# HengyiWang/MorpheuS

Hardware: AMD Instinct MI355X
Metric: rays/sec (fwd+bwd, 128 samples/ray) (higher is better)
Workload: dtype f32 (exact 3 x bf16 operand split on the bf16 MFMA pipe, fp32 accumulate)

## Files before the change

include/morpheus_hip.h:

```cpp
#ifndef MORPHEUS_HIP_H
#define MORPHEUS_HIP_H

#include <stdint.h>

#ifdef __cplusplus
extern "C" {
#endif

#define MH_OK 0
#define MH_ERR_ARG 1
#define MH_ERR_LAUNCH 2
#define MH_ERR_OVERFLOW 3

#define MH_ABI_VERSION 9
#define MH_MAX_LEVELS 32
#define MH_TILE 32

int mh_abi_version(void);
const char *mh_status_string(int status);

int mh_grid_encode_fwd(const float *x, const float *emb, const int32_t *offsets_host,
                       const int32_t *res_host, float *out, int64_t M, int32_t L, int32_t n_levels,
                       float bound, int32_t group, void *stream);
int mh_grid_encode_bwd(const float *grad, const float *x, const float *emb,
// ... 116 lines not shown
int64_t mh_field_wpackT_floats(void);
int mh_field_fwd(const float *xc, const float *feat_s, const float *feat_c, const float *topo,
                 const float *wpack, const float *bias, const float *beta, int32_t n_bands, int32_t with_color,
                 float *sdf, float *sigma, float *albedo, float *acts, int64_t M, void *stream);
int64_t mh_mlp_wgrad_workspace_floats(int32_t n_layers, const int32_t *in_feats_host,
                                      const int32_t *out_feats_host, int64_t n_tiles);
int mh_mlp_wgrad(const float *acts, const float *dpre, int64_t acts_tile_floats, int64_t dpre_tile_floats,
                 int32_t n_layers, const int32_t *act_off_host, const int32_t *dpre_off_host,
                 const int32_t *in_feats_host, const int32_t *out_feats_host, const int32_t *in_live_host,
                 const int32_t *out_live_host, float *workspace, float *dw_raw, float *db_raw, int64_t n_tiles, void *stream);
int mh_mlp_wgrad_b3(const float *acts, const float *dpre, int64_t acts_tile_floats, int64_t dpre_tile_floats,
                    int32_t n_layers, const int32_t *act_off_host, const int32_t *dpre_off_host,
                    const int32_t *in_feats_host, const int32_t *out_feats_host, const int32_t *in_live_host,
                    const int32_t *out_live_host, float *workspace, float *dw_raw, float *db_raw, int64_t n_tiles, void *stream);

int mh_weight_norm_fwd(int32_t n_layers, const float *const *v_host, const float *const *g_host, float *const *w_host,
                       const int32_t *rows_host, const int32_t *cols_host, void *stream);
int mh_weight_norm_bwd(int32_t n_layers, const float *const *v_host, const float *const *g_host,
                       const float *const *dw_host, float *const *dv_host, float *const *dg_host,
                       const int32_t *rows_host, const int32_t *cols_host, void *stream);

int64_t mh_field_bwd_fused_workspace_floats(int64_t M);
int64_t mh_field_dgeo_floats(int64_t M);
int mh_field_bwd_fused(const float *xc, const float *sdf, const float *albedo, const float *g_sdf, const float *g_sigma,
                       const float *g_albedo, const float *wpackT, const float *beta, int32_t n_bands, int32_t with_color,
                       const float *acts, float *dgeo_scratch, float *workspace, float *raw, int32_t accumulate, float *g_xc,
                       float *g_feat_s, float *g_feat_c, float *g_topo, uint32_t *gmax_bits, int64_t M, void *stream);
int64_t mh_field_w3T_bytes(void);
int mh_field_bwd_fused_b3(const float *xc, const float *sdf, const float *albedo, const float *g_sdf, const float *g_sigma,
                          const float *g_albedo, const void *w3T, const float *beta, int32_t n_bands, int32_t with_color,
                          const float *acts, float *dgeo_scratch, float *workspace, float *raw, int32_t accumulate, float *g_xc,
                          float *g_feat_s, float *g_feat_c, float *g_topo, uint32_t *gmax_bits, int64_t M, void *stream);
int64_t mh_field_bwd_pair_min_points(int64_t set);
int mh_adam_step(float *params, const float *grads, float *exp_avg, float *exp_avg_sq, int64_t n, int32_t n_segs,
                 const int64_t *seg_end_host, const float *seg_lr_host, const int64_t *seg_step_host, float beta1,
                 float beta2, float eps, void *stream);
int mh_adam_step_dev(float *params, const float *grads, float *exp_avg, float *exp_avg_sq, int64_t n, int32_t n_segs,
                     const int64_t *seg_end_host, const float *seg_lr_host, const float *seg_flag_dev, int64_t *seg_step_dev,
                     float *seg_scratch_dev, float beta1, float beta2, float eps, void *stream);

int64_t mh_masked_mean_workspace_floats(void);
int mh_masked_mean_fwd(int32_t kind, const float *a, const float *b, const float *w_row, int64_t M, int32_t C,
                       const int32_t *n_valid, float *ws, float *out, void *stream);
int mh_masked_mean_bwd(int32_t kind, const float *a, const float *b, const float *w_row, int64_t M, int32_t C,
                       const int32_t *n_valid, const float *out, const float *g, float *g_a, float *g_b, void *stream);
int mh_ortho_perturb_fwd(const float *x, const float *n, const float *phi, float scale, int64_t M, float *out, void *stream);
int mh_ortho_perturb_bwd(const float *n, const float *phi, const float *g_out, float scale, int64_t M, float *g_n, void *stream);
int mh_smooth_points_fwd(const float *depth, const float *off, const float *rays_o, const float *rays_d, int64_t N, int32_t K,
                         float *pts, float *keep, void *stream);
int mh_smooth_points_bwd(const float *g_pts, const float *depth, const float *off, const float *rays_d, int64_t N, int32_t K,
                         float *g_depth, float *g_o, float *g_d, void *stream);
int mh_bg_blend_fwd(const float *color, const float *opacity, const float *bg, int64_t N, float *image, void *stream);
int mh_bg_blend_bwd(const float *g_image, const float *opacity, const float *bg, int64_t N, float *g_opacity, float *g_bg, void *stream);

int64_t mh_pose_bwd_workspace_floats(int64_t B, int64_t n_per_row);
int mh_pose_apply_fwd(const float *rays_o, const float *rays_d, const float *pose, const int64_t *frame_of_row, int64_t B,
                      int64_t n_per_row, float *o_out, float *d_out, void *stream);
int mh_pose_apply_bwd(const float *rays_d, const float *pose, const int64_t *frame_of_row, int64_t B, int64_t n_per_row,
                      int64_t n_frames, const float *g_o, const float *g_d, float *ws, float *g_pose, void *stream);

int mh_render_loss_fwd(const float *pred_rgb, const float *pred_depth, const float *opacity, const float *image,
                       const float *depth, const float *mask, const float *bg, const float *rays_o, const float *rays_d,
                       int64_t N, float w_rgb, float w_mask, float w_depth, float *gt_rgb, float *valid, float *out, void *stream);
int mh_render_loss_bwd(const float *pred_rgb, const float *pred_depth, const float *opacity, const float *gt_rgb,
                       const float *depth, const float *mask, const float *valid, int64_t N, float w_rgb, float w_mask,
                       float w_depth, const float *g, float *g_rgb, float *g_depth, float *g_opacity, void *stream);
// ... 98 lines not shown
```

morpheus_amd/csrc/mlp.hip:

```cpp
#include "mlp_dev.h"
#include <stdlib.h>
#include <atomic>


__shared__ f32x4 lds_w[4096];

template <int N_F4>
__device__ __forceinline__ void stage_weights(const float *__restrict__ g) {
    static_assert(N_F4 % 256 == 0, "whole rounds of the 256-thread block");
    __syncthreads();
    const f32x4 *src = reinterpret_cast<const f32x4 *>(g);
    const int wave = threadIdx.x >> 6;
#pragma unroll
    for (int k = 0; k < N_F4 / 256; k++)
        __builtin_amdgcn_global_load_lds((const __attribute__((address_space(1))) void *)(src + k * 256 + threadIdx.x),
                                         (__attribute__((address_space(3))) void *)(lds_w + k * 256 + wave * 64), 16, 0, 0);
    asm volatile("s_waitcnt vmcnt(0)" ::: "memory");
    __syncthreads();
}

template <int N_F4>
__device__ __forceinline__ void stage_issue(const float *__restrict__ g) {
    static_assert(N_F4 % 256 == 0, "whole rounds of the 256-thread block");
    const f32x4 *src = reinterpret_cast<const f32x4 *>(g);
// ... 1211 lines not shown
#pragma unroll
        for (int n = 0; n < NI; n++) acc[n] = __builtin_amdgcn_mfma_f32_32x32x16_bf16(as.h[s].h, b[n].m[s].h, acc[n], 0, 0, 0);
#pragma unroll
        for (int n = 0; n < NI; n++) acc[n] = __builtin_amdgcn_mfma_f32_32x32x16_bf16(as.h[s].h, b[n].h[s].h, acc[n], 0, 0, 0);
    }
}
__device__ __forceinline__ void dw_mfma_b3_2(const RowFrag &a, const RowSl *__restrict__ b, f32x16 &acc0, f32x16 &acc1) {
    RowSl as;
    row_slices(a, as);
#pragma unroll
    for (int s = 0; s < 2; s++) {
        acc0 = __builtin_amdgcn_mfma_f32_32x32x16_bf16(as.l[s].h, b[0].h[s].h, acc0, 0, 0, 0);
        acc1 = __builtin_amdgcn_mfma_f32_32x32x16_bf16(as.l[s].h, b[1].h[s].h, acc1, 0, 0, 0);
        acc0 = __builtin_amdgcn_mfma_f32_32x32x16_bf16(as.m[s].h, b[0].m[s].h, acc0, 0, 0, 0);
        acc1 = __builtin_amdgcn_mfma_f32_32x32x16_bf16(as.m[s].h, b[1].m[s].h, acc1, 0, 0, 0);
        acc0 = __builtin_amdgcn_mfma_f32_32x32x16_bf16(as.h[s].h, b[0].l[s].h, acc0, 0, 0, 0);
        acc1 = __builtin_amdgcn_mfma_f32_32x32x16_bf16(as.h[s].h, b[1].l[s].h, acc1, 0, 0, 0);
        acc0 = __builtin_amdgcn_mfma_f32_32x32x16_bf16(as.m[s].h, b[0].h[s].h, acc0, 0, 0, 0);
        acc1 = __builtin_amdgcn_mfma_f32_32x32x16_bf16(as.m[s].h, b[1].h[s].h, acc1, 0, 0, 0);
        acc0 = __builtin_amdgcn_mfma_f32_32x32x16_bf16(as.h[s].h, b[0].m[s].h, acc0, 0, 0, 0);
        acc1 = __builtin_amdgcn_mfma_f32_32x32x16_bf16(as.h[s].h, b[1].m[s].h, acc1, 0, 0, 0);
        acc0 = __builtin_amdgcn_mfma_f32_32x32x16_bf16(as.h[s].h, b[0].h[s].h, acc0, 0, 0, 0);
        acc1 = __builtin_amdgcn_mfma_f32_32x32x16_bf16(as.h[s].h, b[1].h[s].h, acc1, 0, 0, 0);
    }
}
template <int NI>
__device__ __forceinline__ void dw_store_at(float *__restrict__ dw, const f32x16 (&acc)[NI], int mt, int in_pad, int n0, int i, int h) {
#pragma unroll
    for (int n = 0; n < NI; n++)
#pragma unroll
        for (int r = 0; r < 16; r++) dw[(int64_t)(32 * mt + acc_row(r, h)) * in_pad + 32 * (n0 + n) + i] = acc[n][r];
}

__global__ __launch_bounds__(PAIR_THREADS, 1) void field_pair_color_kernel(
    const float *__restrict__ albedo, const float *__restrict__ g_albedo, const float *__restrict__ wpackT,
    const float *__restrict__ acts, float *__restrict__ dgeo_scr, float *__restrict__ g_feat_c, float *__restrict__ ws,
    FusedPart part, uint32_t *__restrict__ gmax, int64_t M, int64_t n_tiles) {
    const int lane = threadIdx.x & 63, wave = __builtin_amdgcn_readfirstlane(threadIdx.x >> 6);
    const int pair = wave & 3, k = wave >> 2;
    const int pt = lane & 31, h = lane >> 5, i = lane & 31;
    constexpr int W_F4 = FUSED_TC2(1) + FUSED_TC1(1) + FUSED_TC0(1);
    stage_pair<W_F4>(wpackT);
    float *scrX = reinterpret_cast<float *>(lds_fused + W_F4) + pair * (2 * SCR_FLOATS), *scrY = scrX + SCR_FLOATS;
    __syncthreads();
    f32x16 w2[1], w1[2][1], w0[2][1], wg[1];
    acc_zero<1>(w2);
    acc_zero<1>(wg);
#pragma unroll
    for (int mt = 0; mt < 2; mt++) {
        acc_zero<1>(w1[mt]);
        acc_zero<1>(w0[mt]);
    }
    float b2 = 0.f, bg = 0.f;
    float b1 = 0.f, b0 = 0.f;
    uint32_t max_c = 0;
    const PairWalk walk = pair_walk(pair, n_tiles);
    RowFrag B[1];
    for (int64_t trip = 0; trip < walk.trips; trip++) {
        const int64_t want = walk.chunk + trip * walk.n_chunks;
        const bool active = want < n_tiles;
        const int64_t tile_id = active ? want : n_tiles - 1;
        const int64_t p = tile_id * TILE + pt;
        const bool live = active && p < M;
        const float *atile = acts + tile_id * (int64_t)(FIELD_ACT_ROWS * TILE);
        const uint32_t *masks = reinterpret_cast<const uint32_t *>(atile + FIELD_HID_ROWS * TILE);
        const f32x4 *wt = lds_fused;
// ... 130 lines not shown
            b0 += q[2 * 64 + lane];
            bg += q[3 * 64 + lane];
        }
    }
    if (pair != 0) return;
    const int64_t pchunk = blockIdx.x;
    dw_store_at<1>(ws + part.dw[2] + pchunk * 32 * 64, w2, 0, 64, k, i, h);
#pragma unroll
    for (int mt = 0; mt < 2; mt++) {
        dw_store_at<1>(ws + part.dw[1] + pchunk * 64 * 64, w1[mt], mt, 64, k, i, h);
        dw_store_at<1>(ws + part.dw[0] + pchunk * 64 * 64, w0[mt], mt, 64, k, i, h);
    }
    dw_store_at<1>(ws + part.dw_s2 + pchunk * 64 * 64, wg, 0, 64, k, i, h);
    if (h == 0) {
        if (k == 0) {
            ws[part.db[2] + pchunk * 32 + i] = b2;
            ws[part.db_s2 + pchunk * 64 + i] = bg;
        }
        ws[part.db[1] + pchunk * 64 + 32 * k + i] = b1;
        ws[part.db[0] + pchunk * 64 + 32 * k + i] = b0;
    }
}

__global__ __launch_bounds__(PAIR_THREADS, 1) void field_pair_sdf_kernel(
    const float *__restrict__ xc, const float *__restrict__ sdf, const float *__restrict__ g_sdf,
    const float *__restrict__ g_sigma, const float *__restrict__ wpackT, const float *__restrict__ beta_p, int n_bands,
    const float *__restrict__ acts, const float *__restrict__ dgeo_scr, float *__restrict__ g_xc,
    float *__restrict__ g_feat_s, float *__restrict__ g_topo, float *__restrict__ ws,
    FusedPart part, uint32_t *__restrict__ gmax, int64_t M, int64_t n_tiles) {
    const int wave = __builtin_amdgcn_readfirstlane(threadIdx.x >> 6);
    const int pair = wave & 3, k = wave >> 2;
    constexpr int W_F4 = FUSED_TS2(1) + FUSED_TS1(1) + FUSED_TS0(1);
    stage_pair<W_F4>(wpackT + 4 * (FUSED_TC2(1) + FUSED_TC1(1) + FUSED_TC0(1)));
    float *scrX = reinterpret_cast<float *>(lds_fused + W_F4) + pair * (2 * SCR_FLOATS), *scrY = scrX + SCR_FLOATS;
    __syncthreads();
    f32x16 w1[2][1], wa[2][1], wb[2];
    acc_zero<2>(wb);
#pragma unroll
    for (int mt = 0; mt < 2; mt++) {
        acc_zero<1>(w1[mt]);
        acc_zero<1>(wa[mt]);
    }
    float wsdf = 0.f;
    float bsdf = 0.f, gb_acc = 0.f;
    float b1 = 0.f, b0 = 0.f;
    uint32_t max_s = 0;
    const float beta = *beta_p;
    const float half_ib2 = __int_as_float(__builtin_amdgcn_readfirstlane(__float_as_int(0.5f / (beta * beta))));
    const float one_ib2 = __int_as_float(__builtin_amdgcn_readfirstlane(__float_as_int(1.0f / (beta * beta))));
    const float one_ib = __int_as_float(__builtin_amdgcn_readfirstlane(__float_as_int(1.0f / beta)));
    const PairWalk walk = pair_walk(pair, n_tiles);
    RowFrag B[2];
    for (int64_t trip = 0; trip < walk.trips; trip++) {
        const int64_t want = walk.chunk + trip * walk.n_chunks;
        const bool active = want < n_tiles;
        const int64_t tile_id = active ? want : n_tiles - 1;
        PAIR_LANE_ANEW;
        const int64_t p = tile_id * TILE + pt;
        const bool live = active && p < M;
        const float *atile = acts + tile_id * (int64_t)(FIELD_ACT_ROWS * TILE);
        const uint32_t *masks = reinterpret_cast<const uint32_t *>(atile + FIELD_HID_ROWS * TILE);
        const f32x4 *wt = lds_fused;
        RowFrag A;
        f32x16 acc[1];
        float own[16];
        float gs = 0.f, gbeta = 0.f;
        if (live && h == 0) {
            const float s = sdf[p];
            if (g_sdf) gs = g_sdf[p];
            if (g_sigma) {
                const float gsg = g_sigma[p];
                const float sg = (s > 0.f) ? 1.f : ((s < 0.f) ? -1.f : 0.f);
                const float a = fabsf(s) / beta;
                const float ex = expf(-a);
                gs += gsg * (-half_ib2 * sg * sg * ex);
                gbeta = gsg * (-one_ib2 * laplace_unit(s, beta) + one_ib * (0.5f * sg * ex * (fabsf(s) / (beta * beta))));
            }
        }
        gb_acc += gbeta;
        const uint32_t mw1 = masks[1 * 64 + lane] >> (16 * k), mw0 = masks[0 * 64 + lane] >> (16 * k);
        float d2[32];
        {
            const f32x4 *gsrc = reinterpret_cast<const f32x4 *>(dgeo_scr + (tile_id * 64 + lane) * 16);
#pragma unroll
            for (int q = 0; q < 4; q++) {
                const f32x4 v = gsrc[q];
#pragma unroll
                for (int c = 0; c < 4; c++) d2[4 * q + c] = active ? v[c] : 0.f;
            }
        }
#pragma unroll
        for (int r = 0; r < 16; r++) d2[16 + r] = 0.f;
        d2[16] = gs;
        row_load_async(B[0], atile, 160 + 32 * k + i, h);
        mfma_tiles_z_b3<32, 2, 1, 3>(wt, k, d2, acc, lane);
        wt += FUSED_TS2(1);
#pragma unroll
        for (int r = 0; r < 16; r++) own[r] = mask_bit(mw1, r, acc[0][r]);
        fused_wait<1>(B);
#pragma unroll
        for (int j = 0; j < 4; j++)
#pragma unroll
            for (int q = 0; q < 4; q++) {
                const float g = __shfl(gs, 16 * h + 4 * j + q);
                wsdf = fmaf(g, B[0].v[j][q], wsdf);
                bsdf += g;
            }
        asm volatile("" : "+v"(wsdf), "+v"(bsdf));
        __builtin_amdgcn_sched_barrier(0);
        {
            PAIR_LANE_ANEW;
            RowSl Bs[1];
            row_load_async(B[0], atile, 96 + 32 * k + i, h);
            scr_put_tile(scrX, own, k, pt, h);
            __syncthreads();
            mfma_tiles_scr_b3<2, 1>(wt, k, scrX, pt, h, acc, lane);
            wt += FUSED_TS1(1);
#pragma unroll
            for (int r = 0; r < 16; r++) own[r] = mask_bit(mw0, r, acc[0][r]);
            fused_wait<1>(B);
            row_slices(B[0], Bs[0]);
#pragma unroll
            for (int mt = 0; mt < 2; mt++) {
                scr_get(A, scrX, 32 * mt + i, h);
                if (k == mt) dw_bias(A, b1);
                dw_mfma_b3<1>(A, Bs, w1[mt]);
            }
            __builtin_amdgcn_sched_barrier(0);
        }
        {
            PAIR_LANE_ANEW;
            row_load_async(B[0], atile, k == 0 ? 64 + min(i, 15) : i, h);
            row_load_async(B[1], atile, k == 0 ? 64 + min(i, 15) : 32 + i, h);
            scr_put_tile(scrY, own, k, pt, h);
        }
        __syncthreads();
        if (k == 0) {
            PAIR_LANE_ANEW;
            const int64_t p = tile_id * TILE + pt;
            const bool live = active && p < M;
            RowSl Bs[1];
            f32x16(&e)[2] = wb;
            mfma_tiles_scr_b3<3, 2>(wt, 0, scrY, pt, h, e, lane);
            float gx[3] = {0.f, 0.f, 0.f};
            if (g_xc) {
                float dsc[18];
                enc_deriv_parked(atile, pt, h, dsc);
#pragma unroll
                for (int kk = 0; kk < 18; kk++) {
                    const float de = kk < 16 ? e[0][kk] : e[1][kk - 16];
                    gx[kk % 3] += de * dsc[kk];
                }
                if (h == 0) {
                    gx[0] += e[1][2];
                    gx[2] += e[1][3];
                } else {
                    gx[1] += e[1][2];
                }
#pragma unroll
                for (int d = 0; d < 3; d++) gx[d] += __shfl_xor(gx[d], 32);
            }
            if (live) {
                if (g_xc && h == 0) {
                    g_xc[p * 3 + 0] = gx[0];
                    g_xc[p * 3 + 1] = gx[1];
                    g_xc[p * 3 + 2] = gx[2];
                }
                if (g_topo) g_topo[p * 2 + h] = e[1][4];
            }
            __builtin_amdgcn_sched_barrier(0);
            fused_wait<2>(B);
            row_slices(B[0], Bs[0]);
#pragma unroll
            for (int mt = 0; mt < 2; mt++) {
                scr_get(A, scrY, 32 * mt + i, h);
                if (mt == 0) dw_bias(A, b0);
                dw_mfma_b3<1>(A, Bs, wa[mt]);
                __builtin_amdgcn_sched_barrier(0);
            }
            __builtin_amdgcn_sched_barrier(0);
        } else {
            PAIR_LANE_ANEW;
            const int64_t p = tile_id * TILE + pt;
            const bool live = active && p < M;
            RowSl Bs[2];
            f32x16 e[1];
            mfma_tiles_scr_b3<3, 1>(wt, 2, scrY, pt, h, e, lane);
            if (live && g_feat_s) {
                f32x4 *o = reinterpret_cast<f32x4 *>(g_feat_s + p * 32 + 16 * h);
#pragma unroll
                for (int q = 0; q < 4; q++) {
                    f32x4 v;
#pragma unroll
                    for (int c = 0; c < 4; c++) v[c] = e[0][4 * q + c];
                    o[q] = v;
                }
#pragma unroll
                for (int r = 0; r < 16; r++) max_s = max(max_s, __float_as_uint(fabsf(e[0][r])));
            }
            __builtin_amdgcn_sched_barrier(0);
            fused_wait<2>(B);
            row_slices(B[0], Bs[0]);
            row_slices(B[1], Bs[1]);
#pragma unroll
            for (int mt = 0; mt < 2; mt++) {
                scr_get(A, scrY, 32 * mt + i, h);
                if (mt == 1) dw_bias(A, b0);
                dw_mfma_b3_2(A, Bs, wa[mt][0], wb[mt]);
                __builtin_amdgcn_sched_barrier(0);
            }
            __builtin_amdgcn_sched_barrier(0);
        }
    }
    const int lane = __lane_id(), h = lane >> 5, i = lane & 31;
    if (gmax) {
#pragma unroll
        for (int o = 32; o > 0; o >>= 1) max_s = max(max_s, (uint32_t)__shfl_xor((int)max_s, o));
        if (lane == 0 && max_s) atomicMax(gmax + 0, max_s);
    }
    wsdf += __shfl_xor(wsdf, 32);
    bsdf += __shfl_xor(bsdf, 32);
    b1 += __shfl_xor(b1, 32);
    b0 += __shfl_xor(b0, 32);
    float *red = reinterpret_cast<float *>(lds_fused) + k * PAIR_RED_FLOATS;
    for (int src = 1; src < 4; src++) {
        __syncthreads();
        if (pair == src) {
            float *q = acc_to_lds<1>(w1[0], red, lane);
            q = acc_to_lds<1>(w1[1], q, lane);
            q = acc_to_lds<1>(wa[0], q, lane);
            q = acc_to_lds<1>(wa[1], q, lane);
            if (k == 1) acc_to_lds<2>(wb, q, lane);
            q += 2 * 1024;
            q[0 * 64 + lane] = bsdf;
            q[1 * 64 + lane] = b1;
            q[2 * 64 + lane] = b0;
            q[3 * 64 + lane] = wsdf;
            q[4 * 64 + lane] = gb_acc;
        }
        __syncthreads();
        if (pair == 0) {
// ... 960 lines not shown
    const WarpWg w = warp_wg_geometry();
    WgRegenHost rg;
    for (int k = 0; k < WG_MAX_LAYERS; k++) rg.on[k] = false;
    rg.M = M;
    for (int net = 0; net < 2; net++) {
        const int k = net * 6 + 4;
        rg.on[k] = regen_dpre4 != 0;
        rg.g5[k] = net ? g_topo : g_deform;
        rg.nout[k] = net ? 2 : 3;
        rg.w3T[k] = reinterpret_cast<const f32x4 *>(net ? w3T_t : w3T_d);
        rg.mask_off[k] = WARP_HID_ROWS * TILE + (net * 5 + 4) * 64 * 2;
    }
    return wgrad_impl(acts, dpre, (int64_t)WARP_ACT_ROWS * TILE, (int64_t)WARP_DPRE_ROWS * TILE, 12, w.act_off, w.dpre_off, w.in, w.out,
                      w.in_live, w.out_live, workspace, dw_raw, db_raw, n_tiles_for(M), stream, true, regen_dpre4 ? &rg : nullptr);
}

static const int FUSED_IN[6] = {96, 64, 64, 64, 64, 64};
static const int FUSED_OUT[6] = {64, 64, 64, 64, 64, 32};

static inline int fused_blocks(int64_t n_tiles) {
    const int64_t need = (n_tiles + FUSED_THREADS / 64 - 1) / (FUSED_THREADS / 64);
    const int64_t cus = mh_cu_count();
    return (int)(need < cus ? need : cus);
}

extern "C" int64_t mh_field_bwd_fused_workspace_floats(int64_t M) {
    const int64_t chunks = (int64_t)fused_blocks(n_tiles_for(M));
    int64_t per = 0;
    for (int l = 0; l < 6; l++) per += (int64_t)FUSED_IN[l] * FUSED_OUT[l] + FUSED_OUT[l];
    return chunks * (per + 1);
}
extern "C" int64_t mh_field_dgeo_floats(int64_t M) { return n_tiles_for(M) * 64 * 16; }

static std::atomic<int64_t> g_pair_min_points{0};
extern "C" int64_t mh_field_bwd_pair_min_points(int64_t set) {
    if (set >= 0) g_pair_min_points.store(set, std::memory_order_relaxed);
    return g_pair_min_points.load(std::memory_order_relaxed);
}

static int field_bwd_fused_impl(const float *xc, const float *sdf, const float *albedo, const float *g_sdf,
                                const float *g_sigma, const float *g_albedo, const float *wpackT, const float *beta,
                                int32_t n_bands, int32_t with_color, const float *acts, float *dgeo_scratch,
                                float *workspace, float *raw, int32_t accumulate, float *g_xc, float *g_feat_s, float *g_feat_c,
                                float *g_topo, uint32_t *gmax_bits, int64_t M, void *stream, bool b3) {
    if (M == 0) return MH_OK;
    if (M < 0 || !xc || !sdf || !wpackT || !acts || !workspace || !raw || n_bands < 0 || n_bands > 6 || !beta) return MH_ERR_ARG;
    if (with_color && (!albedo || !dgeo_scratch)) return MH_ERR_ARG;
    static MhOncePerDevice opted;
    const size_t lds_c = (size_t)(FUSED_TC2(b3) + FUSED_TC1(b3) + FUSED_TC0(b3)) * 16 + (size_t)(4 * SCR_FLOATS) * sizeof(float);
    const size_t lds_s = (size_t)(FUSED_TS2(b3) + FUSED_TS1(b3) + FUSED_TS0(b3)) * 16 + (size_t)(4 * SCR_FLOATS) * sizeof(float);
    const size_t pair_lds_c = (size_t)(FUSED_TC2(1) + FUSED_TC1(1) + FUSED_TC0(1)) * 16 + (size_t)(8 * SCR_FLOATS) * sizeof(float);
    const size_t pair_lds_s = (size_t)(FUSED_TS2(1) + FUSED_TS1(1) + FUSED_TS0(1)) * 16 + (size_t)(8 * SCR_FLOATS) * sizeof(float);
    static_assert((FUSED_TS2(1) + FUSED_TS1(1) + FUSED_TS0(1)) * 16 + 8 * SCR_FLOATS * 4 <= 160 * 1024, "pair form: LDS of one CU");
    const bool pair = b3 && with_color && M >= g_pair_min_points.load(std::memory_order_relaxed);
    const int dev = mh_device();
    if (opted.need(dev)) {
        const int big_c = (int)((size_t)(FUSED_TC2(1) + FUSED_TC1(1) + FUSED_TC0(1)) * 16 + (size_t)(4 * SCR_FLOATS) * sizeof(float));
        const int big_s = (int)((size_t)(FUSED_TS2(1) + FUSED_TS1(1) + FUSED_TS0(1)) * 16 + (size_t)(4 * SCR_FLOATS) * sizeof(float));
        if (hipFuncSetAttribute((const void *)field_fused_color_kernel<false>, hipFuncAttributeMaxDynamicSharedMemorySize, big_c) != hipSuccess ||
            hipFuncSetAttribute((const void *)field_fused_color_kernel<true>, hipFuncAttributeMaxDynamicSharedMemorySize, big_c) != hipSuccess ||
            hipFuncSetAttribute((const void *)field_fused_sdf_kernel<true, false>, hipFuncAttributeMaxDynamicSharedMemorySize, big_s) != hipSuccess ||
            hipFuncSetAttribute((const void *)field_fused_sdf_kernel<false, false>, hipFuncAttributeMaxDynamicSharedMemorySize, big_s) != hipSuccess ||
            hipFuncSetAttribute((const void *)field_fused_sdf_kernel<true, true>, hipFuncAttributeMaxDynamicSharedMemorySize, big_s) != hipSuccess ||
            hipFuncSetAttribute((const void *)field_fused_sdf_kernel<false, true>, hipFuncAttributeMaxDynamicSharedMemorySize, big_s) != hipSuccess ||
            hipFuncSetAttribute((const void *)field_pair_color_kernel, hipFuncAttributeMaxDynamicSharedMemorySize, (int)pair_lds_c) != hipSuccess ||
            hipFuncSetAttribute((const void *)field_pair_sdf_kernel, hipFuncAttributeMaxDynamicSharedMemorySize, (int)pair_lds_s) != hipSuccess)
            return MH_ERR_LAUNCH;
        opted.mark(dev);
    }
    const int64_t n_tiles = n_tiles_for(M);
    const int blocks = fused_blocks(n_tiles);
    const int64_t chunks = blocks;
    int64_t dw_off[6], db_off[6], off = 0, dw_total = 0, db_total = 0;
    for (int l = 0; l < 6; l++) {
        dw_off[l] = off;
        off += chunks * FUSED_IN[l] * FUSED_OUT[l];
        dw_total += (int64_t)FUSED_IN[l] * FUSED_OUT[l];
    }
    for (int l = 0; l < 6; l++) {
        db_off[l] = off;
        off += chunks * FUSED_OUT[l];
        db_total += FUSED_OUT[l];
    }
    FusedPart pc, ps;
    for (int k = 0; k < 3; k++) {
        ps.dw[k] = dw_off[k];
        ps.db[k] = db_off[k];
        pc.dw[k] = dw_off[3 + k];
        pc.db[k] = db_off[3 + k];
    }
    ps.gb = off;
    pc.gb = off;
    ps.dw_s2 = pc.dw_s2 = dw_off[2];
    ps.db_s2 = pc.db_s2 = db_off[2];
    hipStream_t st = mh_stream(stream);
#define FUSED_LAUNCH_COLOR(B3_)                                                                                             \
    hipLaunchKernelGGL(field_fused_color_kernel<B3_>, dim3((unsigned)blocks), dim3(FUSED_THREADS), lds_c, st, albedo, g_albedo, wpackT, \
                       acts, dgeo_scratch, g_feat_c, workspace, pc, gmax_bits, M, n_tiles)
#define FUSED_LAUNCH_SDF(WC, B3_, DGEO)                                                                                      \
    hipLaunchKernelGGL((field_fused_sdf_kernel<WC, B3_>), dim3((unsigned)blocks), dim3(FUSED_THREADS), lds_s, st, xc, sdf, g_sdf, \
                       g_sigma, wpackT, beta, (int)n_bands, acts, (const float *)(DGEO), g_xc, g_feat_s, g_topo,             \
                       workspace, ps, gmax_bits, M, n_tiles)
    if (pair) {
        hipLaunchKernelGGL(field_pair_color_kernel, dim3((unsigned)blocks), dim3(PAIR_THREADS), pair_lds_c, st, albedo, g_albedo, wpackT,
                           acts, dgeo_scratch, g_feat_c, workspace, pc, gmax_bits, M, n_tiles);
        MH_CHECK_LAUNCH();
        hipLaunchKernelGGL(field_pair_sdf_kernel, dim3((unsigned)blocks), dim3(PAIR_THREADS), pair_lds_s, st, xc, sdf, g_sdf, g_sigma,
                           wpackT, beta, (int)n_bands, acts, (const float *)dgeo_scratch, g_xc, g_feat_s, g_topo, workspace, ps,
                           gmax_bits, M, n_tiles);
    } else if (with_color) {
        if (b3) FUSED_LAUNCH_COLOR(true); else FUSED_LAUNCH_COLOR(false);
        MH_CHECK_LAUNCH();
        if (b3) FUSED_LAUNCH_SDF(true, true, dgeo_scratch); else FUSED_LAUNCH_SDF(true, false, dgeo_scratch);
    } else {
        if (b3) FUSED_LAUNCH_SDF(false, true, nullptr); else FUSED_LAUNCH_SDF(false, false, nullptr);
    }
#undef FUSED_LAUNCH_COLOR
#undef FUSED_LAUNCH_SDF
    MH_CHECK_LAUNCH();
    const int n_l = with_color ? 6 : 3;
    WgReduce rd;
    rd.n = 13;
    rd.accumulate = accumulate ? 1 : 0;
    int64_t dw_out = 0, db_out = 0;
    rd.first[0] = 0;
    for (int l = 0; l < 6; l++) {
        const int32_t ch = l < n_l ? (int32_t)chunks : 0;
        rd.chunks[l] = ch;
        rd.len[l] = FUSED_IN[l] * FUSED_OUT[l];
        rd.part_off[l] = dw_off[l];
        rd.out_off[l] = dw_out;
        rd.chunks[6 + l] = ch;
        rd.len[6 + l] = FUSED_OUT[l];
        rd.part_off[6 + l] = db_off[l];
        rd.out_off[6 + l] = dw_total + db_out;
        dw_out += (int64_t)FUSED_IN[l] * FUSED_OUT[l];
        db_out += FUSED_OUT[l];
    }
    rd.chunks[12] = (int32_t)chunks;
    rd.len[12] = 1;
    rd.part_off[12] = ps.gb;
    rd.out_off[12] = dw_total + db_total;
    for (int sgm = 0; sgm < rd.n; sgm++) rd.first[sgm + 1] = rd.first[sgm] + rd.len[sgm];
    const int64_t total = rd.first[rd.n];
    hipLaunchKernelGGL(wgrad_reduce_kernel, dim3((unsigned)((total + 63) / 64)), dim3(256), 0, st, workspace, raw, rd);
    MH_CHECK_LAUNCH();
// ... 36 lines not shown
```

morpheus_amd/ops.py:

```python
from __future__ import annotations

import ctypes
import math
import os
from typing import Optional, Sequence

import numpy as np
import torch

from . import _lib
from ._lib import check, launch, ptr, require_gpu, stream
from .packing import field_joint_packer, field_packer, warp_joint_packer, warp_packer



class KernelTimer:

    def __init__(self):
        self.enabled = False
        self.records = {}
        self._pool, self._used = [], 0

    def reset(self, enabled: bool):
        self.enabled, self.records, self._used = enabled, {}, 0
# ... 944 lines not shown
    act_off, dpre_off, in_pad, out_pad, in_live, out_live = [], [], [], [], [], []
    for net in range(2):
        for l in range(6):
            act_off.append(0 if l == 0 else (64 + net * 640 + (l - 1) * 128) * 32)
            dpre_off.append((net * 672 + l * 128) * 32)
            in_pad.append(64 if l == 0 else 128)
            out_pad.append(32 if l == 5 else 128)
            in_live.append(40 if l == 0 else 128)
            out_live.append((3, 2)[net] if l == 5 else 128)
    return act_off, dpre_off, in_pad, out_pad, in_live, out_live


_WARP_WG = _warp_wg_geometry()

def warp_mlp(x, slot, bias0_d, bias0_t, n_bands, opnd: MLPOperands, slots_are_identity: bool = False):
    return _WarpMLP.apply(x, slot, bias0_d, bias0_t, opnd.token, n_bands, opnd, slots_are_identity)


def _field_fwd(lib, xc, fs, fc, tp, beta_c, n_bands, with_color, opnd, need_grad):
    w, b = opnd.w[0], opnd.b[0]
    M, dev = xc.shape[0], xc.device
    acts = _scratch(lib.mh_field_acts_floats(M), dev) if need_grad else None
    sdf, sigma = torch.empty(M, device=dev), torch.empty(M, device=dev)
    albedo = torch.empty(M, 3, device=dev) if with_color else None
    if opnd.w3 is not None:
        _timed("mh_field_fwd_b3", ptr(xc), ptr(fs), ptr(fc), ptr(tp), ptr(opnd.w3[0]), ptr(b), ptr(beta_c), n_bands,
               int(bool(with_color)), ptr(sdf), ptr(sigma), ptr(albedo), ptr(acts), M, key="mh_field_fwd")
    else:
        _timed("mh_field_fwd", ptr(xc), ptr(fs), ptr(fc), ptr(tp), ptr(w), ptr(b), ptr(beta_c), n_bands, int(bool(with_color)),
               ptr(sdf), ptr(sigma), ptr(albedo), ptr(acts), M)
    return sdf, sigma, albedo, acts


FIELD_BWD = os.environ.get("MORPHEUS_FIELD_BWD", "b3")
if FIELD_BWD not in ("b3", "b3w1", "sdf", "f32"):
    raise ValueError(f"MORPHEUS_FIELD_BWD={FIELD_BWD!r}: expected 'b3', 'b3w1', 'sdf' or 'f32'")
_PAIR_NEVER = 1 << 62
_pair_min_default = None


def _field_wT(opnd, with_color: bool):
    sliced = FIELD_BWD in ("b3", "b3w1") or (FIELD_BWD == "sdf" and not with_color)
    if sliced and opnd.mode == "b3" and opnd.wT3 is not None:
        return opnd.wT3[0], True
    return opnd.wT[0], False


def _field_bwd(lib, xc, wT, beta_c, acts, sdf, albedo, g_sdf, g_sigma, g_albedo, n_bands, with_color, has_topo, has_fc,
               need_dx, jp, raw_into=None, gmax=None, b3=False):
    M, dev = xc.shape[0], xc.device
    if not with_color:
        g_albedo = None
    g_xc = torch.empty(M, 3, device=dev) if need_dx else None
    g_fs = _scratch(M * 32, dev).view(M, 32)
    g_fc = _scratch(M * 32, dev).view(M, 32) if (with_color and has_fc) else None
    g_tp = torch.empty(M, 2, device=dev) if has_topo else None
    if gmax is None:
        gmax = torch.zeros(2, dtype=torch.int32, device=dev)
    dgeo = _scratch(lib.mh_field_dgeo_floats(M), dev) if with_color else None
    ws = torch.empty(lib.mh_field_bwd_fused_workspace_floats(M), device=dev)
    raw = None
    if raw_into is None:
        raw = torch.empty(jp.raw_len + 1, device=dev) if M > 0 else torch.zeros(jp.raw_len + 1, device=dev)
    c = lambda t: None if t is None else t.contiguous()
    if b3 and with_color:
        global _pair_min_default
        if _pair_min_default is None:
            _pair_min_default = lib.mh_field_bwd_pair_min_points(-1)
        want = _PAIR_NEVER if FIELD_BWD == "b3w1" else _pair_min_default
        if lib.mh_field_bwd_pair_min_points(-1) != want:
            lib.mh_field_bwd_pair_min_points(want)
    _timed("mh_field_bwd_fused_b3" if b3 else "mh_field_bwd_fused", ptr(xc), ptr(sdf), ptr(albedo if with_color else None), ptr(c(g_sdf)),
           ptr(c(g_sigma)), ptr(c(g_albedo)), ptr(wT), ptr(beta_c), n_bands, int(with_color), ptr(acts), ptr(dgeo), ptr(ws),
           ptr(raw) if raw_into is None else ctypes.c_void_p(raw_into), int(raw_into is not None), ptr(g_xc), ptr(g_fs), ptr(g_fc),
           ptr(g_tp), ptr(gmax), M, key="mh_field_bwd_fused")
    return g_xc, g_fs, g_fc, g_tp, raw, gmax


class _FieldMLP(torch.autograd.Function):

    @staticmethod
    def forward(ctx, xc, feat_s, feat_c, topo, beta, token, n_bands, with_color, opnd):
        ctx.set_materialize_grads(False)
        require_gpu(xc, feat_s, feat_c, topo, beta)
        lib = _lib.load()
        xc = xc.detach().contiguous().float()
        fs = feat_s.detach().contiguous()
        fc = None if feat_c is None else feat_c.detach().contiguous()
        tp = None if topo is None else topo.detach().contiguous()
        beta_c = beta.detach().reshape(1).contiguous().float()
        sdf, sigma, albedo, acts = _field_fwd(lib, xc, fs, fc, tp, beta_c, n_bands, with_color, opnd, any(ctx.needs_input_grad))
        wT_sel, ctx.bwd_b3 = _field_wT(opnd, bool(with_color))
        ctx.save_for_backward(xc, wT_sel, beta_c, acts, sdf, albedo)
        ctx.cfg = (n_bands, bool(with_color), topo is not None, feat_c is not None)
        ctx.jp = opnd.jp
        if albedo is None:
            albedo = torch.empty(0, device=xc.device)
            ctx.mark_non_differentiable(albedo)
        return sdf, sigma, albedo

    @staticmethod
    def backward(ctx, g_sdf, g_sigma, g_albedo):
        lib = _lib.load()
        xc, wT, beta_c, acts, sdf, albedo = ctx.saved_tensors
# ... 388 lines not shown
```

Measured before the change: 1.074 million.

## Store pair SDF kernel scratch as pre-split bf16 planes read via transpose loads

The pair SDF backward kernel now writes activation tiles into LDS as three pre-split bf16 planes (high/mid/low) instead of fp32 scratch. Forward MFMAs read the planes directly and the weight-gradient MFMAs fetch them with ds_read_tr16 transposed loads, so the fp32-to-bf16 split is not recomputed on each read. This cuts LDS footprint per pair and split work, at the cost of an extra barrier before reusing the single plane buffer. Separately, the pair colour kernel gets its own threshold, disabled by default, so the default path now pairs only the SDF kernel with the non-pair colour kernel.

```diff
diff --git a/include/morpheus_hip.h b/include/morpheus_hip.h
--- a/include/morpheus_hip.h
+++ b/include/morpheus_hip.h
@@ -172,6 +172,7 @@
                           const float *acts, float *dgeo_scratch, float *workspace, float *raw, int32_t accumulate, float *g_xc,
                           float *g_feat_s, float *g_feat_c, float *g_topo, uint32_t *gmax_bits, int64_t M, void *stream);
 int64_t mh_field_bwd_pair_min_points(int64_t set);
+int64_t mh_field_bwd_pair_color_min_points(int64_t set);
 int mh_adam_step(float *params, const float *grads, float *exp_avg, float *exp_avg_sq, int64_t n, int32_t n_segs,
                  const int64_t *seg_end_host, const float *seg_lr_host, const int64_t *seg_step_host, float beta1,
                  float beta2, float eps, void *stream);
diff --git a/morpheus_amd/csrc/mlp.hip b/morpheus_amd/csrc/mlp.hip
--- a/morpheus_amd/csrc/mlp.hip
+++ b/morpheus_amd/csrc/mlp.hip
@@ -1267,6 +1267,132 @@
         for (int r = 0; r < 16; r++) dw[(int64_t)(32 * mt + acc_row(r, h)) * in_pad + 32 * (n0 + n) + i] = acc[n][r];
 }
 
+#define PLN_ROWB 144
+#define PLN_BYTES (32 * PLN_ROWB)
+#define PAIR_PLN_BYTES (3 * PLN_BYTES)
+typedef short s16x4 __attribute__((ext_vector_type(4)));
+
+__device__ __forceinline__ void pln_put_tile(char *__restrict__ pl, const float (&v)[16], int k, int pt, int h) {
+    char *dst = pl + pt * PLN_ROWB + (8 * k + 2 * h) * 8;
+#pragma unroll
+    for (int u = 0; u < 2; u++) {
+        Frag fh, fm, fl;
+#pragma unroll
+        for (int e2 = 0; e2 < 4; e2++) split2(v[8 * u + 2 * e2], v[8 * u + 2 * e2 + 1], fh.u[e2], fm.u[e2], fl.u[e2]);
+        *reinterpret_cast<f32x4 *>(dst + 0 * PLN_BYTES + 32 * u) = fh.f;
+        *reinterpret_cast<f32x4 *>(dst + 1 * PLN_BYTES + 32 * u) = fm.f;
+        *reinterpret_cast<f32x4 *>(dst + 2 * PLN_BYTES + 32 * u) = fl.f;
+    }
+}
+
+template <int MT, int NT>
+__device__ __forceinline__ void mfma_tiles_pln_b3(const f32x4 *__restrict__ w, int t0, const char *__restrict__ pl, int pt, int h,
+                                                  f32x16 (&acc)[NT], int lane) {
+    constexpr int S = 4, PL = MT * S * 64;
+    const f32x16 zero = {0.f, 0.f, 0.f, 0.f, 0.f, 0.f, 0.f, 0.f, 0.f, 0.f, 0.f, 0.f, 0.f, 0.f, 0.f, 0.f};
+    w += t0 * S * 64 + lane;
+    pl += pt * PLN_ROWB + 16 * h;
+#pragma unroll
+    for (int s = 0; s < S; s++) {
+        Frag bh, bm, bl;
+        bh.f = *reinterpret_cast<const f32x4 *>(pl + 0 * PLN_BYTES + 32 * s);
+        bm.f = *reinterpret_cast<const f32x4 *>(pl + 1 * PLN_BYTES + 32 * s);
+        bl.f = *reinterpret_cast<const f32x4 *>(pl + 2 * PLN_BYTES + 32 * s);
+        Frag ah[NT], am[NT], al[NT];
+#pragma unroll
+        for (int t = 0; t < NT; t++) {
+            ah[t].f = w[0 * PL + (t * S + s) * 64];
+            am[t].f = w[1 * PL + (t * S + s) * 64];
+            al[t].f = w[2 * PL + (t * S + s) * 64];
+        }
+#pragma unroll
+        for (int t = 0; t < NT; t++) acc[t] = __builtin_amdgcn_mfma_f32_32x32x16_bf16(al[t].h, bh.h, s == 0 ? zero : acc[t], 0, 0, 0);
+#pragma unroll
+        for (int t = 0; t < NT; t++) acc[t] = __builtin_amdgcn_mfma_f32_32x32x16_bf16(am[t].h, bm.h, acc[t], 0, 0, 0);
+#pragma unroll
+        for (int t = 0; t < NT; t++) acc[t] = __builtin_amdgcn_mfma_f32_32x32x16_bf16(ah[t].h, bl.h, acc[t], 0, 0, 0);
+#pragma unroll
+        for (int t = 0; t < NT; t++) acc[t] = __builtin_amdgcn_mfma_f32_32x32x16_bf16(am[t].h, bh.h, acc[t], 0, 0, 0);
+#pragma unroll
+        for (int t = 0; t < NT; t++) acc[t] = __builtin_amdgcn_mfma_f32_32x32x16_bf16(ah[t].h, bm.h, acc[t], 0, 0, 0);
+#pragma unroll
+        for (int t = 0; t < NT; t++) acc[t] = __builtin_amdgcn_mfma_f32_32x32x16_bf16(ah[t].h, bh.h, acc[t], 0, 0, 0);
+        __builtin_amdgcn_sched_barrier(0);
+    }
+}
+
+__device__ __forceinline__ void pln_get(RowSl &as, const char *__restrict__ pl, int mt, int lane) {
+    const int G = lane >> 4, j = (lane >> 2) & 3, q = lane & 3;
+    const char *src = pl + (16 * (G >> 1) + j) * PLN_ROWB + (8 * mt + 4 * (G & 1) + 2 * (q & 1) + (q >> 1)) * 8;
+#pragma unroll
+    for (int s = 0; s < 2; s++)
+#pragma unroll
+        for (int t = 0; t < 2; t++) {
+            union {
+                s16x4 v;
+                uint32_t u[2];
+            } ch, cm, cl;
+            const char *a = src + (8 * s + 4 * t) * PLN_ROWB;
+            ch.v = __builtin_amdgcn_ds_read_tr16_b64_v4i16((__attribute__((address_space(3))) s16x4 *)(a + 0 * PLN_BYTES));
+            cm.v = __builtin_amdgcn_ds_read_tr16_b64_v4i16((__attribute__((address_space(3))) s16x4 *)(a + 1 * PLN_BYTES));
+            cl.v = __builtin_amdgcn_ds_read_tr16_b64_v4i16((__attribute__((address_space(3))) s16x4 *)(a + 2 * PLN_BYTES));
+#pragma unroll
+            for (int c = 0; c < 2; c++) {
+                as.h[s].u[2 * t + c] = ch.u[c];
+                as.m[s].u[2 * t + c] = cm.u[c];
+                as.l[s].u[2 * t + c] = cl.u[c];
+            }
+        }
+}
+__device__ __forceinline__ void dw_bias_sl(const RowSl &as, float &bsum) {
+#pragma unroll
+    for (int j = 0; j < 4; j++) {
+        float a[4];
+#pragma unroll
+        for (int c = 0; c < 2; c++) {
+            const uint32_t uh = as.h[j >> 1].u[2 * (j & 1) + c], um = as.m[j >> 1].u[2 * (j & 1) + c], ul = as.l[j >> 1].u[2 * (j & 1) + c];
+            a[2 * c] = (__uint_as_float(uh << 16) + __uint_as_float(um << 16)) + __uint_as_float(ul << 16);
+            a[2 * c + 1] = (__uint_as_float(uh & 0xffff0000u) + __uint_as_float(um & 0xffff0000u)) + __uint_as_float(ul & 0xffff0000u);
+        }
+        bsum += (a[0] + a[1]) + (a[2] + a[3]);
+    }
+}
+template <int NI>
+__device__ __forceinline__ void dw_mfma_sl(const RowSl &as, const RowSl *__restrict__ b, f32x16 (&acc)[NI]) {
+#pragma unroll
+    for (int s = 0; s < 2; s++) {
+#pragma unroll
+        for (int n = 0; n < NI; n++) acc[n] = __builtin_amdgcn_mfma_f32_32x32x16_bf16(as.l[s].h, b[n].h[s].h, acc[n], 0, 0, 0);
+#pragma unroll
+        for (int n = 0; n < NI; n++) acc[n] = __builtin_amdgcn_mfma_f32_32x32x16_bf16(as.m[s].h, b[n].m[s].h, acc[n], 0, 0, 0);
+#pragma unroll
+        for (int n = 0; n < NI; n++) acc[n] = __builtin_amdgcn_mfma_f32_32x32x16_bf16(as.h[s].h, b[n].l[s].h, acc[n], 0, 0, 0);
+#pragma unroll
+        for (int n = 0; n < NI; n++) acc[n] = __builtin_amdgcn_mfma_f32_32x32x16_bf16(as.m[s].h, b[n].h[s].h, acc[n], 0, 0, 0);
+#pragma unroll
+        for (int n = 0; n < NI; n++) acc[n] = __builtin_amdgcn_mfma_f32_32x32x16_bf16(as.h[s].h, b[n].m[s].h, acc[n], 0, 0, 0);
+#pragma unroll
+        for (int n = 0; n < NI; n++) acc[n] = __builtin_amdgcn_mfma_f32_32x32x16_bf16(as.h[s].h, b[n].h[s].h, acc[n], 0, 0, 0);
+    }
+}
+__device__ __forceinline__ void dw_mfma_sl_2(const RowSl &as, const RowSl *__restrict__ b, f32x16 &acc0, f32x16 &acc1) {
+#pragma unroll
+    for (int s = 0; s < 2; s++) {
+        acc0 = __builtin_amdgcn_mfma_f32_32x32x16_bf16(as.l[s].h, b[0].h[s].h, acc0, 0, 0, 0);
+        acc1 = __builtin_amdgcn_mfma_f32_32x32x16_bf16(as.l[s].h, b[1].h[s].h, acc1, 0, 0, 0);
+        acc0 = __builtin_amdgcn_mfma_f32_32x32x16_bf16(as.m[s].h, b[0].m[s].h, acc0, 0, 0, 0);
+        acc1 = __builtin_amdgcn_mfma_f32_32x32x16_bf16(as.m[s].h, b[1].m[s].h, acc1, 0, 0, 0);
+        acc0 = __builtin_amdgcn_mfma_f32_32x32x16_bf16(as.h[s].h, b[0].l[s].h, acc0, 0, 0, 0);
+        acc1 = __builtin_amdgcn_mfma_f32_32x32x16_bf16(as.h[s].h, b[1].l[s].h, acc1, 0, 0, 0);
+        acc0 = __builtin_amdgcn_mfma_f32_32x32x16_bf16(as.m[s].h, b[0].h[s].h, acc0, 0, 0, 0);
+        acc1 = __builtin_amdgcn_mfma_f32_32x32x16_bf16(as.m[s].h, b[1].h[s].h, acc1, 0, 0, 0);
+        acc0 = __builtin_amdgcn_mfma_f32_32x32x16_bf16(as.h[s].h, b[0].m[s].h, acc0, 0, 0, 0);
+        acc1 = __builtin_amdgcn_mfma_f32_32x32x16_bf16(as.h[s].h, b[1].m[s].h, acc1, 0, 0, 0);
+        acc0 = __builtin_amdgcn_mfma_f32_32x32x16_bf16(as.h[s].h, b[0].h[s].h, acc0, 0, 0, 0);
+        acc1 = __builtin_amdgcn_mfma_f32_32x32x16_bf16(as.h[s].h, b[1].h[s].h, acc1, 0, 0, 0);
+    }
+}
+
 __global__ __launch_bounds__(PAIR_THREADS, 1) void field_pair_color_kernel(
     const float *__restrict__ albedo, const float *__restrict__ g_albedo, const float *__restrict__ wpackT,
     const float *__restrict__ acts, float *__restrict__ dgeo_scr, float *__restrict__ g_feat_c, float *__restrict__ ws,
@@ -1463,7 +1589,7 @@
     const int pair = wave & 3, k = wave >> 2;
     constexpr int W_F4 = FUSED_TS2(1) + FUSED_TS1(1) + FUSED_TS0(1);
     stage_pair<W_F4>(wpackT + 4 * (FUSED_TC2(1) + FUSED_TC1(1) + FUSED_TC0(1)));
-    float *scrX = reinterpret_cast<float *>(lds_fused + W_F4) + pair * (2 * SCR_FLOATS), *scrY = scrX + SCR_FLOATS;
+    char *pln = reinterpret_cast<char *>(lds_fused + W_F4) + pair * PAIR_PLN_BYTES;
     __syncthreads();
     f32x16 w1[2][1], wa[2][1], wb[2];
     acc_zero<2>(wb);
@@ -1492,7 +1618,6 @@
         const float *atile = acts + tile_id * (int64_t)(FIELD_ACT_ROWS * TILE);
         const uint32_t *masks = reinterpret_cast<const uint32_t *>(atile + FIELD_HID_ROWS * TILE);
         const f32x4 *wt = lds_fused;
-        RowFrag A;
         f32x16 acc[1];
         float own[16];
         float gs = 0.f, gbeta = 0.f;
@@ -1543,9 +1668,10 @@
             PAIR_LANE_ANEW;
             RowSl Bs[1];
             row_load_async(B[0], atile, 96 + 32 * k + i, h);
-            scr_put_tile(scrX, own, k, pt, h);
             __syncthreads();
-            mfma_tiles_scr_b3<2, 1>(wt, k, scrX, pt, h, acc, lane);
+            pln_put_tile(pln, own, k, pt, h);
+            __syncthreads();
+            mfma_tiles_pln_b3<2, 1>(wt, k, pln, pt, h, acc, lane);
             wt += FUSED_TS1(1);
 #pragma unroll
             for (int r = 0; r < 16; r++) own[r] = mask_bit(mw0, r, acc[0][r]);
@@ -1553,9 +1679,10 @@
             row_slices(B[0], Bs[0]);
 #pragma unroll
             for (int mt = 0; mt < 2; mt++) {
-                scr_get(A, scrX, 32 * mt + i, h);
-                if (k == mt) dw_bias(A, b1);
-                dw_mfma_b3<1>(A, Bs, w1[mt]);
+                RowSl As;
+                pln_get(As, pln, mt, lane);
+                if (k == mt) dw_bias_sl(As, b1);
+                dw_mfma_sl<1>(As, Bs, w1[mt]);
             }
             __builtin_amdgcn_sched_barrier(0);
         }
@@ -1563,7 +1690,8 @@
             PAIR_LANE_ANEW;
             row_load_async(B[0], atile, k == 0 ? 64 + min(i, 15) : i, h);
             row_load_async(B[1], atile, k == 0 ? 64 + min(i, 15) : 32 + i, h);
-            scr_put_tile(scrY, own, k, pt, h);
+            __syncthreads();
+            pln_put_tile(pln, own, k, pt, h);
         }
         __syncthreads();
         if (k == 0) {
@@ -1572,7 +1700,7 @@
             const bool live = active && p < M;
             RowSl Bs[1];
             f32x16(&e)[2] = wb;
-            mfma_tiles_scr_b3<3, 2>(wt, 0, scrY, pt, h, e, lane);
+            mfma_tiles_pln_b3<3, 2>(wt, 0, pln, pt, h, e, lane);
             float gx[3] = {0.f, 0.f, 0.f};
             if (g_xc) {
                 float dsc[18];
@@ -1604,9 +1732,10 @@
             row_slices(B[0], Bs[0]);
 #pragma unroll
             for (int mt = 0; mt < 2; mt++) {
-                scr_get(A, scrY, 32 * mt + i, h);
-                if (mt == 0) dw_bias(A, b0);
-                dw_mfma_b3<1>(A, Bs, wa[mt]);
+                RowSl As;
+                pln_get(As, pln, mt, lane);
+                if (mt == 0) dw_bias_sl(As, b0);
+                dw_mfma_sl<1>(As, Bs, wa[mt]);
                 __builtin_amdgcn_sched_barrier(0);
             }
             __builtin_amdgcn_sched_barrier(0);
@@ -1616,7 +1745,7 @@
             const bool live = active && p < M;
             RowSl Bs[2];
             f32x16 e[1];
-            mfma_tiles_scr_b3<3, 1>(wt, 2, scrY, pt, h, e, lane);
+            mfma_tiles_pln_b3<3, 1>(wt, 2, pln, pt, h, e, lane);
             if (live && g_feat_s) {
                 f32x4 *o = reinterpret_cast<f32x4 *>(g_feat_s + p * 32 + 16 * h);
 #pragma unroll
@@ -1635,9 +1764,10 @@
             row_slices(B[1], Bs[1]);
 #pragma unroll
             for (int mt = 0; mt < 2; mt++) {
-                scr_get(A, scrY, 32 * mt + i, h);
-                if (mt == 1) dw_bias(A, b0);
-                dw_mfma_b3_2(A, Bs, wa[mt][0], wb[mt]);
+                RowSl As;
+                pln_get(As, pln, mt, lane);
+                if (mt == 1) dw_bias_sl(As, b0);
+                dw_mfma_sl_2(As, Bs, wa[mt][0], wb[mt]);
                 __builtin_amdgcn_sched_barrier(0);
             }
             __builtin_amdgcn_sched_barrier(0);
@@ -2664,10 +2794,16 @@
 }
 extern "C" int64_t mh_field_dgeo_floats(int64_t M) { return n_tiles_for(M) * 64 * 16; }
 
+#define PAIR_NEVER ((int64_t)1 << 62)
 static std::atomic<int64_t> g_pair_min_points{0};
+static std::atomic<int64_t> g_pair_color_min_points{PAIR_NEVER};
 extern "C" int64_t mh_field_bwd_pair_min_points(int64_t set) {
     if (set >= 0) g_pair_min_points.store(set, std::memory_order_relaxed);
     return g_pair_min_points.load(std::memory_order_relaxed);
+}
+extern "C" int64_t mh_field_bwd_pair_color_min_points(int64_t set) {
+    if (set >= 0) g_pair_color_min_points.store(set, std::memory_order_relaxed);
+    return g_pair_color_min_points.load(std::memory_order_relaxed);
 }
 
 static int field_bwd_fused_impl(const float *xc, const float *sdf, const float *albedo, const float *g_sdf,
@@ -2682,9 +2818,12 @@
     const size_t lds_c = (size_t)(FUSED_TC2(b3) + FUSED_TC1(b3) + FUSED_TC0(b3)) * 16 + (size_t)(4 * SCR_FLOATS) * sizeof(float);
     const size_t lds_s = (size_t)(FUSED_TS2(b3) + FUSED_TS1(b3) + FUSED_TS0(b3)) * 16 + (size_t)(4 * SCR_FLOATS) * sizeof(float);
     const size_t pair_lds_c = (size_t)(FUSED_TC2(1) + FUSED_TC1(1) + FUSED_TC0(1)) * 16 + (size_t)(8 * SCR_FLOATS) * sizeof(float);
-    const size_t pair_lds_s = (size_t)(FUSED_TS2(1) + FUSED_TS1(1) + FUSED_TS0(1)) * 16 + (size_t)(8 * SCR_FLOATS) * sizeof(float);
-    static_assert((FUSED_TS2(1) + FUSED_TS1(1) + FUSED_TS0(1)) * 16 + 8 * SCR_FLOATS * 4 <= 160 * 1024, "pair form: LDS of one CU");
-    const bool pair = b3 && with_color && M >= g_pair_min_points.load(std::memory_order_relaxed);
+    const size_t pair_lds_s = (size_t)(FUSED_TS2(1) + FUSED_TS1(1) + FUSED_TS0(1)) * 16 + (size_t)(4 * PAIR_PLN_BYTES);
+    static_assert((FUSED_TS2(1) + FUSED_TS1(1) + FUSED_TS0(1)) * 16 + 4 * PAIR_PLN_BYTES <= 160 * 1024, "pair form: LDS of one CU");
+    static_assert((FUSED_TC2(1) + FUSED_TC1(1) + FUSED_TC0(1)) * 16 + 8 * SCR_FLOATS * 4 <= 160 * 1024, "pair form: LDS of one CU");
+    static_assert(2 * PAIR_RED_FLOATS * 4 <= (FUSED_TS2(1) + FUSED_TS1(1) + FUSED_TS0(1)) * 16, "the end-of-kernel sum lives in the packs' area");
+    const bool pair_s = b3 && with_color && M >= g_pair_min_points.load(std::memory_order_relaxed);
+    const bool pair_c = b3 && with_color && M >= g_pair_color_min_points.load(std::memory_order_relaxed);
     const int dev = mh_device();
     if (opted.need(dev)) {
         const int big_c = (int)((size_t)(FUSED_TC2(1) + FUSED_TC1(1) + FUSED_TC0(1)) * 16 + (size_t)(4 * SCR_FLOATS) * sizeof(float));
@@ -2733,17 +2872,19 @@
     hipLaunchKernelGGL((field_fused_sdf_kernel<WC, B3_>), dim3((unsigned)blocks), dim3(FUSED_THREADS), lds_s, st, xc, sdf, g_sdf, \
                        g_sigma, wpackT, beta, (int)n_bands, acts, (const float *)(DGEO), g_xc, g_feat_s, g_topo,             \
                        workspace, ps, gmax_bits, M, n_tiles)
-    if (pair) {
-        hipLaunchKernelGGL(field_pair_color_kernel, dim3((unsigned)blocks), dim3(PAIR_THREADS), pair_lds_c, st, albedo, g_albedo, wpackT,
-                           acts, dgeo_scratch, g_feat_c, workspace, pc, gmax_bits, M, n_tiles);
+    if (with_color) {
+        if (pair_c)
+            hipLaunchKernelGGL(field_pair_color_kernel, dim3((unsigned)blocks), dim3(PAIR_THREADS), pair_lds_c, st, albedo, g_albedo, wpackT,
+                               acts, dgeo_scratch, g_feat_c, workspace, pc, gmax_bits, M, n_tiles);
+        else if (b3) FUSED_LAUNCH_COLOR(true);
+        else FUSED_LAUNCH_COLOR(false);
         MH_CHECK_LAUNCH();
-        hipLaunchKernelGGL(field_pair_sdf_kernel, dim3((unsigned)blocks), dim3(PAIR_THREADS), pair_lds_s, st, xc, sdf, g_sdf, g_sigma,
-                           wpackT, beta, (int)n_bands, acts, (const float *)dgeo_scratch, g_xc, g_feat_s, g_topo, workspace, ps,
-                           gmax_bits, M, n_tiles);
-    } else if (with_color) {
-        if (b3) FUSED_LAUNCH_COLOR(true); else FUSED_LAUNCH_COLOR(false);
-        MH_CHECK_LAUNCH();
-        if (b3) FUSED_LAUNCH_SDF(true, true, dgeo_scratch); else FUSED_LAUNCH_SDF(true, false, dgeo_scratch);
+        if (pair_s)
+            hipLaunchKernelGGL(field_pair_sdf_kernel, dim3((unsigned)blocks), dim3(PAIR_THREADS), pair_lds_s, st, xc, sdf, g_sdf, g_sigma,
+                               wpackT, beta, (int)n_bands, acts, (const float *)dgeo_scratch, g_xc, g_feat_s, g_topo, workspace, ps,
+                               gmax_bits, M, n_tiles);
+        else if (b3) FUSED_LAUNCH_SDF(true, true, dgeo_scratch);
+        else FUSED_LAUNCH_SDF(true, false, dgeo_scratch);
     } else {
         if (b3) FUSED_LAUNCH_SDF(false, true, nullptr); else FUSED_LAUNCH_SDF(false, false, nullptr);
     }
diff --git a/morpheus_amd/ops.py b/morpheus_amd/ops.py
--- a/morpheus_amd/ops.py
+++ b/morpheus_amd/ops.py
@@ -1000,15 +1000,17 @@
     return sdf, sigma, albedo, acts
 
 
+_PAIR_FORMS = {"b3": (None, None), "b3w1": (False, False), "b3w2": (True, True), "b3c2": (True, False), "b3s2": (False, True)}
 FIELD_BWD = os.environ.get("MORPHEUS_FIELD_BWD", "b3")
-if FIELD_BWD not in ("b3", "b3w1", "sdf", "f32"):
-    raise ValueError(f"MORPHEUS_FIELD_BWD={FIELD_BWD!r}: expected 'b3', 'b3w1', 'sdf' or 'f32'")
+if FIELD_BWD not in tuple(_PAIR_FORMS) + ("sdf", "f32"):
+    raise ValueError(f"MORPHEUS_FIELD_BWD={FIELD_BWD!r}: expected 'b3', 'b3w1', 'b3w2', 'b3c2', 'b3s2', 'sdf' or 'f32'")
 _PAIR_NEVER = 1 << 62
 _pair_min_default = None
+_pair_color_min_default = None
 
 
 def _field_wT(opnd, with_color: bool):
-    sliced = FIELD_BWD in ("b3", "b3w1") or (FIELD_BWD == "sdf" and not with_color)
+    sliced = FIELD_BWD in _PAIR_FORMS or (FIELD_BWD == "sdf" and not with_color)
     if sliced and opnd.mode == "b3" and opnd.wT3 is not None:
         return opnd.wT3[0], True
     return opnd.wT[0], False
@@ -1032,12 +1034,16 @@
         raw = torch.empty(jp.raw_len + 1, device=dev) if M > 0 else torch.zeros(jp.raw_len + 1, device=dev)
     c = lambda t: None if t is None else t.contiguous()
     if b3 and with_color:
-        global _pair_min_default
+        global _pair_min_default, _pair_color_min_default
         if _pair_min_default is None:
             _pair_min_default = lib.mh_field_bwd_pair_min_points(-1)
-        want = _PAIR_NEVER if FIELD_BWD == "b3w1" else _pair_min_default
-        if lib.mh_field_bwd_pair_min_points(-1) != want:
-            lib.mh_field_bwd_pair_min_points(want)
+            _pair_color_min_default = lib.mh_field_bwd_pair_color_min_points(-1)
+        pair_c, pair_s = _PAIR_FORMS[FIELD_BWD]
+        for knob, pair, default in ((lib.mh_field_bwd_pair_color_min_points, pair_c, _pair_color_min_default),
+                                    (lib.mh_field_bwd_pair_min_points, pair_s, _pair_min_default)):
+            want = default if pair is None else (0 if pair else _PAIR_NEVER)
+            if knob(-1) != want:
+                knob(want)
     _timed("mh_field_bwd_fused_b3" if b3 else "mh_field_bwd_fused", ptr(xc), ptr(sdf), ptr(albedo if with_color else None), ptr(c(g_sdf)),
            ptr(c(g_sigma)), ptr(c(g_albedo)), ptr(wT), ptr(beta_c), n_bands, int(with_color), ptr(acts), ptr(dgeo), ptr(ws),
            ptr(raw) if raw_into is None else ctypes.c_void_p(raw_into), int(raw_into is not None), ptr(g_xc), ptr(g_fs), ptr(g_fc),
```

Result: no change. 1.079 million (median of 6 runs) (+0.5%).
